# NVlabs/long-video-gan

Measured on NVIDIA H100. Metric: frames/sec (G+D train step: every convolution and torch_utils.ops call of the forward/backward passes, replayed), higher is better.
Workload: dtype f32

## Files before the change

### include/lvg_ops.h

```cpp
#ifndef LVG_OPS_H_
#define LVG_OPS_H_

#include <stdint.h>

#ifdef __cplusplus
extern "C" {
#endif

#define LVG_ABI_VERSION 2

#define LVG_OK            0
#define LVG_UNSUPPORTED (-1)
#define LVG_ERR_ARG       1
#define LVG_ERR_CUDA      2

#define LVG_F32 0
#define LVG_F16 1
#define LVG_F64 2

#define LVG_ACT_LINEAR   1
#define LVG_ACT_RELU     2
#define LVG_ACT_LRELU    3
#define LVG_ACT_TANH     4
#define LVG_ACT_SIGMOID  5
#define LVG_ACT_ELU      6
#define LVG_ACT_SELU     7
#define LVG_ACT_SOFTPLUS 8
#define LVG_ACT_SWISH    9

int         lvg_abi_version(void);
const char* lvg_last_error(void);
const char* lvg_build_info(void);
int64_t     lvg_launch_count(void);

int lvg_bias_act(const void* x, const void* b, const void* xref, const void* yref,
                 const void* dy, void* y, int dtype, int64_t n, int64_t size_b,
                 int64_t step_b, int grad, int act, float alpha, float gain,
                 float clamp, void* stream);

int lvg_bias_act_grad_db(const void* dy_in, const void* b, const void* xref,
                         const void* yref, void* dx, float* db_f32, int dtype,
                         int64_t n, int64_t size_b, int64_t step_b, int act,
                         float alpha, float gain, float clamp, void* stream);
int lvg_bias_act_fwd_codes(const void* x, const void* b, void* y, void* codes, int dtype, int64_t n,
                           int64_t size_b, int64_t step_b, int act, float alpha, float gain, float clamp,
                           void* stream);
int lvg_bias_act_bwd_codes(const void* dy, const void* codes, void* dx, float* db_f32, int dtype, int64_t n,
                           int64_t size_b, int64_t step_b, int act, float alpha, float gain, float clamp,
                           void* stream);
int64_t lvg_bias_act_codes_bytes(int dtype, int64_t n);

int lvg_upfirdn2d(const void* x, const float* f, void* y, int dtype,
                  const int64_t x_shape[4], const int64_t x_stride[4],
                  const int64_t y_shape[4], const int64_t y_stride[4],
                  int fw, int fh, int64_t f_stride_x, int64_t f_stride_y,
                  int upx, int upy, int downx, int downy, int padx0, int pady0,
                  int flip, float gain, void* stream);

int lvg_upfirdn2d_sep(const void* x, const float* fx, const float* fy, void* y,
                      int dtype, const int64_t x_shape[4], const int64_t x_stride[4],
                      const int64_t y_shape[4], const int64_t y_stride[4],
                      int fw, int fh, int upx, int upy, int downx, int downy,
                      int padx0, int pady0, int flip, float gain, void* stream);

int lvg_filtered_lrelu(const void* x, const float* fu, const float* fd, const void* b,
                       const uint8_t* si, void* y, uint8_t* so, int dtype,
                       const int64_t x_shape[4], const int64_t x_stride[4],
                       const int64_t y_shape[4], const int64_t y_stride[4],
                       int fu_w, int fu_h, int fd_w, int fd_h, int up, int down,
                       int px0, int py0, int s_h, int s_wbytes, int sx, int sy,
                       float gain, float slope, float clamp, int flip,
                       int write_signs, void* stream);

int lvg_filtered_lrelu_supported(int dtype, int fu_w, int fu_h, int fd_w, int fd_h,
                                 int up, int down);

int lvg_filtered_lrelu_act(void* x, const uint8_t* si, uint8_t* so, int dtype,
                           const int64_t x_shape[4], const int64_t x_stride[4],
                           int s_h, int s_wbytes, int sx, int sy, float gain,
                           float slope, float clamp, int write_signs, void* stream);

int lvg_fma(const void* a, const void* b, const void* c, void* out, int dtype,
            int rank, const int64_t shape[6], const int64_t a_stride[6],
            const int64_t b_stride[6], const int64_t c_stride[6], void* stream);

int64_t lvg_convnd_workspace(int dtype, int n, int groups, int cin, int cout, int t, int h, int wd,
                             int kt, int kh, int kw, int pad_t, int pad_h, int pad_w);
int lvg_convnd_fprop(const void* x, const void* w, void* y, int dtype, int n, int groups, int cin, int cout,
                     int t, int h, int wd, int kt, int kh, int kw, int pad_t, int pad_h, int pad_w, int stride,
                     const float* bias, int act, float alpha, float gain, float clamp,
                     void* workspace, int64_t workspace_bytes, void* stream);
int lvg_convnd_dgrad(const void* dy, const void* w, void* dx, int dtype, int n, int groups, int cin, int cout,
                     int t, int h, int wd, int kt, int kh, int kw, int pad_t, int pad_h, int pad_w, int stride,
                     void* workspace, int64_t workspace_bytes, void* stream);
int64_t lvg_convnd_wgrad_workspace(int dtype, int n, int groups, int cin, int cout, int t, int h, int wd,
                                   int kt, int kh, int kw, int pad_t, int pad_h, int pad_w);
int lvg_convnd_wgrad(const void* x, const void* dy, void* dw, int dtype, int n, int groups, int cin, int cout,
                     int t, int h, int wd, int kt, int kh, int kw, int pad_t, int pad_h, int pad_w, int stride,
                     void* workspace, int64_t workspace_bytes, void* stream);
int lvg_convnd_plan(int mode, int dtype, int n, int groups, int cin, int cout, int t, int h, int wd, int kt, int kh, int kw,
                    int pad_t, int pad_h, int pad_w, int stride, int* out, int out_len);
int lvg_convnd_epilogue_plan(int mode, int dtype, int n, int groups, int cin, int cout, int t, int h, int wd, int kt, int kh,
                             int kw, int pad_t, int pad_h, int pad_w, int stride, int* out, int out_len);
int lvg_convnd_route(int mode, int dtype, int n, int groups, int cin, int cout, int t, int h, int wd, int kt, int kh, int kw,
                     int pad_t, int pad_h, int pad_w, int stride, int epilogue);
int lvg_convnd_wgrad_plan(int dtype, int n, int groups, int cin, int cout, int t, int h, int wd, int kt, int kh, int kw,
                          int pad_t, int pad_h, int pad_w, int* out, int out_len);
int64_t lvg_convnd_backward_workspace(int dtype, int n, int groups, int cin, int cout, int t, int h, int wd,
                                      int kt, int kh, int kw, int pad_t, int pad_h, int pad_w);
int lvg_convnd_backward(const void* x, const void* dy, const void* w, void* dx, void* dw, int dtype, int n, int groups,
                        int cin, int cout, int t, int h, int wd, int kt, int kh, int kw, int pad_t, int pad_h, int pad_w,
                        int stride, void* workspace, int64_t workspace_bytes, void* stream);

int64_t lvg_modconv_workspace(int dtype, int n, int cin, int cout, int t, int h, int wd, int kt, int kh, int kw,
                              int pad_t, int pad_h, int pad_w);
int lvg_modconv_fprop(const void* x, const void* w, const float* a, const float* d, void* y, int dtype, int n, int cin,
                      int cout, int t, int h, int wd, int kt, int kh, int kw, int pad_t, int pad_h, int pad_w,
                      void* workspace, int64_t workspace_bytes, void* stream);
int lvg_modconv_backward(const void* x, const void* w, const float* a, const float* d, const void* y, const void* dy,
                         void* dx, void* dw, float* da, float* dyy, int dtype, int n, int cin, int cout, int t, int h,
                         int wd, int kt, int kh, int kw, int pad_t, int pad_h, int pad_w, void* workspace,
                         int64_t workspace_bytes, void* stream);

int64_t lvg_fir1d_depthwise_workspace(int groups);
int lvg_fir1d_depthwise(const float* x, const float* w, float* y, int n, int groups, int lin, int k,
                        void* workspace, int64_t workspace_bytes, void* stream);

int lvg_fir3d(const void* x, const float* f, void* y, int dtype, int n, int c, int t_in, int h_in, int w_in, int t_out,
              int h_out, int w_out, int filt_t, int filt_h, int filt_w, int step_t, int step_h, int step_w, int off_t,
              int off_h, int off_w, int fold, void* stream);
int lvg_fir3d_adjoint(const void* x, const float* f, void* y, int dtype, int n, int c, int t_in, int h_in, int w_in,
                      int t_out, int h_out, int w_out, int filt_t, int filt_h, int filt_w, int step_t, int step_h,
                      int step_w, int off_t, int off_h, int off_w, int fold, void* stream);

#define LVG_VIDEO_AUGMENT_LINEAR 1
int64_t lvg_video_augment_workspace(int n, int c, int t_in, int h, int w, int t_out);
int lvg_video_augment(const float* x, const float* params, float* y, void* workspace, int n, int c, int t_in, int h, int w,
                      int t_out, int flags, void* stream);
int lvg_video_augment_adjoint(const float* dy, const float* params, float* dx, void* workspace, int n, int c, int t_in,
                              int h, int w, int t_out, void* stream);

#define LVG_AUGMENT_PIPE_NPAR 23
#define LVG_AUGMENT_PIPE_GEOM 1
#define LVG_AUGMENT_PIPE_LINEAR 2
int64_t lvg_augment_pipe_workspace(int n, int c, int t, int h, int w, int flags);
int lvg_augment_pipe(const float* x, const float* params, const float* filter, int ntaps, const float* noise, float* y, int n,
                     int c, int t, int h, int w, int flags, void* stream);
int lvg_augment_pipe_adjoint(const float* dy, const float* params, const float* filter, int ntaps, float* dx, void* workspace,
                             int n, int c, int t, int h, int w, int flags, void* stream);

#define LVG_GBLOCK_TAIL_TUP 1
#define LVG_GBLOCK_TAIL_SUP 2
int64_t lvg_gblock_tail_workspace(int n, int c, int t, int h, int w, int t_out, int h_out, int w_out, int flags);
int lvg_gblock_tail(const void* s, const void* h, const float* b, void* z, uint8_t* codes, int dtype, int n, int c, int t,
                    int hh, int ww, int t_out, int h_out, int w_out, int flags, int act, float alpha, float gain, float clamp,
                    void* stream);
int lvg_gblock_tail_adjoint(const void* dz, const uint8_t* codes, void* dm, float* db, void* workspace, int64_t workspace_bytes,
                            int dtype, int n, int c, int t, int hh, int ww, int t_out, int h_out, int w_out, int flags, int act,
                            float alpha, float gain, void* stream);

#define LVG_DBLOCK_TAIL_TDOWN 1
#define LVG_DBLOCK_TAIL_SDOWN 2
#define LVG_DBLOCK_TAIL_MERGE 4
#define LVG_DBLOCK_TAIL_NONE 0
#define LVG_DBLOCK_TAIL_WRITE 1
#define LVG_DBLOCK_TAIL_READ 2
int64_t lvg_dblock_tail_workspace(int n, int c, int t, int h, int w, int flags);
int64_t lvg_dblock_tail_codes_bytes(int n, int c, int t, int h, int w, int flags);
int lvg_dblock_tail(const void* y, const void* s, const float* b, const float* f, void* z, uint8_t* codes, int mode, int dtype,
                    int n, int c, int t, int h, int w, int flags, int act, float alpha, float gain, float clamp, void* stream);
int lvg_dblock_tail_adjoint(const void* dz, const uint8_t* codes, const float* f, void* dy, void* ds, float* db, void* workspace,
                            int64_t workspace_bytes, int dtype, int n, int c, int t, int h, int w, int flags, int act,
                            float alpha, float gain, void* stream);

#define LVG_SRES_COND_NPLAN 10
int64_t lvg_sres_cond_workspace(int n, int t, int c, int c_lr, int window, int t_lr, int h_lr, int w_lr, int z_dtype,
                                const int* plan_h, const int* plan_w);
int lvg_sres_cond(const void* x, const float* lr, const float* f_h, const float* f_w, void* z, float* mean_sq, void* workspace,
                  int64_t workspace_bytes, int x_dtype, int z_dtype, int n, int t, int c, int c_lr, int window, int t_lr,
                  int h_lr, int w_lr, const int64_t* lr_strides, const int* plan_h, const int* plan_w, float gain_h,
                  float gain_w, void* stream);

int64_t lvg_sres_layer_workspace(int dtype, int n, int t, int c, int c_lr, int window, int t_lr, int h_lr, int w_lr,
                                 const int* plan_h, const int* plan_w, int cout, int kh, int kw, int pad_h, int pad_w);
int lvg_sres_layer_fprop(const void* x, const float* lr, const float* f_h, const float* f_w, const void* w, const float* a,
                         const float* d, void* y, float* mean_sq, int x_dtype, int dtype, int n, int t, int c, int c_lr,
                         int window, int t_lr, int h_lr, int w_lr, const int64_t* lr_strides, const int* plan_h,
                         const int* plan_w, float gain_h, float gain_w, int cout, int kh, int kw, int pad_h, int pad_w,
                         void* workspace, int64_t workspace_bytes, void* stream);
int lvg_sres_layer_backward(const void* x, const float* lr, const float* f_h, const float* f_w, const void* w, const float* a,
// ... 67 lines not shown
```

### long-video-gan_b200/csrc/conv_engine.cuh

```cuda
#pragma once

#include <cuda_bf16.h>

#include "common.cuh"

namespace lvg {

__device__ __forceinline__ unsigned short bf16_bits(float v) { return __bfloat16_as_ushort(__float2bfloat16_rn(v)); }
__device__ __forceinline__ float bf16_val(unsigned short b) { return __uint_as_float((uint32_t)b << 16); }

__device__ __forceinline__ float to_f32(float v) { return v; }
__device__ __forceinline__ float to_f32(__half v) { return __half2float(v); }
__device__ __forceinline__ void from_f32(float& o, float v) { o = v; }
__device__ __forceinline__ void from_f32(__half& o, float v) { o = __float2half_rn(v); }

inline int round_up(int a, int b) { return (a + b - 1) / b * b; }
inline int64_t round256(int64_t b) { return (b + 255) / 256 * 256; }

struct ConvShape {
    int dtype, n, groups, cin, cout, t, h, wd, kt, kh, kw, pad_t, pad_h, pad_w, stride;

    int split() const { return dtype == LVG_F32 ? 1 : 0; }
    int taps() const { return kt * kh * kw; }
    int64_t inst() const { return (int64_t)n * groups; }
    int64_t thw() const { return (int64_t)t * h * wd; }
    int to() const { return t + 2 * pad_t - kt + 1; }
    int ho() const { return h + 2 * pad_h - kh + 1; }
    int wo() const { return wd + 2 * pad_w - kw + 1; }
    int hos() const { return (ho() - 1) / stride + 1; }
    int wos() const { return (wo() - 1) / stride + 1; }
    bool empty() const { return to() < 1 || ho() < 1 || wo() < 1; }

    bool tileable() const;
    bool fprop_ok() const;
    bool dgrad_ok() const;
    bool wgrad_ok() const;
};

struct Geometry {
    int cpad, cblk, nblk, nimg, kc, mt;
    int m64, a_img;
    int64_t act_bytes, w_bytes;
};
Geometry geometry(int split, int64_t inst, int groups, int ck, int cm, int64_t thw, int taps);

struct ActGate {
    const void* y;
    int act;
    float alpha, gain, clamp;
};

struct IgemmJob {
    const void* x;
    const unsigned char* x8_pre;
    const float* in_scale;
    ActGate in_gate;
    int xin_h, xin_w, dil;
    int dtype, n, groups, ck, cm, t, h, wd, kt, kh, kw, pad_t, pad_h, pad_w;
    const void* w;
    int64_t gs, sm, sk;
    int flip;
    void* y;
    const float* bias;
    int act;
    float alpha, gain, clamp;
    const float* out_scale;
    int ostride;
};
IgemmJob fprop_job(const ConvShape& s, const void* x, const void* w, void* y);
IgemmJob dgrad_job(const ConvShape& s, const void* dy, const void* w, void* dx);

struct IgemmRooms {
    int64_t wp, x8;
    int64_t total() const { return wp + x8 + 256; }
};
IgemmRooms igemm_rooms(const IgemmJob& j);
int run_igemm(const IgemmJob& j, void* workspace, int64_t workspace_bytes, cudaStream_t s);

struct WgradPlan {
    int split, cpad_a, cpad_b, nt, ntiles, mt, nsplit;
    int ablk, khc, mrows;
    int nseg, seg_w[4], seg_x0[4], ps, rh, stages;
    int a_stage, b_stage, stage_bytes, tail_bytes;
    size_t smem;
    int64_t a_bytes, b_bytes, part_bytes, dw_elems;
};
WgradPlan wgrad_plan(const ConvShape& s, bool fold = true);

struct WgradInputs {
    const unsigned char* dy8_pre;
    const unsigned char* x8_pre;
    const float* x_scale;
    const float* dy_scale;
    ActGate dy_gate;
};

struct WgradRooms {
    int64_t dy8, x8, part;
    int64_t total() const { return dy8 + x8 + part + 512; }
};
WgradRooms wgrad_rooms(const WgradPlan& q, bool dy8_pre);
int run_wgrad(const ConvShape& s, const void* x, const void* dy, void* dw, const WgradInputs& in, void* workspace, int64_t workspace_bytes,
              cudaStream_t st);

struct BackwardRooms {
    int64_t dy8, rest;
    int64_t x8;
    int64_t total() const { return dy8 + rest; }
};
bool shares_dy8(const ConvShape& s);
BackwardRooms backward_rooms(const ConvShape& s, bool shared);
int64_t backward_workspace(const ConvShape& s);
struct Backward {
    const unsigned char* dy8;
    unsigned char* rest;
    int64_t rest_bytes;
    unsigned char* x8;
    ActGate gate;
};
int backward_dgrad(const ConvShape& s, const void* dy, const float* d, const void* w, void* dx, void* workspace, int64_t workspace_bytes,
                   cudaStream_t st, Backward& b, const ActGate* gate = nullptr);
int backward_wgrad(const ConvShape& s, const Backward& b, const void* x, const void* dy, const float* d, void* dw, const float* x_scale,
                   const unsigned char* x8_pre, cudaStream_t st);

bool modconv_in_envelope(const ConvShape& s);
int modconv_rowdot(void* u, const void* v, const float* scale, float* r, int dtype, int64_t rows, int64_t len, cudaStream_t s);

}
```

### long-video-gan_b200/csrc/conv_igemm.cu

```cuda

#include <algorithm>
#include <cuda.h>
#include <stdlib.h>
#include <type_traits>

#include "common.cuh"
#include "wgmma.cuh"
#include "conv_engine.cuh"

namespace lvg {
bool pw_supported(int dtype, int groups, int cin, int cout, int kt, int kh, int kw, int pad_t, int pad_h, int pad_w, int stride, int64_t P);
int pw_conv(const float* x, const float* w, float* y, int n, int cin, int cout, int64_t P, int64_t w_sco, int64_t w_sci, cudaStream_t s);
bool pw_tc_supported(int dtype, int groups, int cin, int cout, int kt, int kh, int kw, int pad_t, int pad_h, int pad_w, int stride, int64_t P);
int pw_tc_conv(const void* x, const void* w, void* y, int dtype, int n, int ck, int cm, int64_t P, int64_t w_sm, int64_t w_sk, void* workspace,
               int64_t workspace_bytes, cudaStream_t s, const void* res = nullptr, float rscale = 1.f);
int64_t pw_tc_workspace(int dtype, int ck, int cm);
}

namespace lvg {
namespace {

using namespace tc;

constexpr int kBM = 128;
// ... 827 lines not shown
    int nt;
    int nblk_a, nblk_b;
    int lo_a, lo_b;
    int nseg, seg_w[4], seg_x0[4], ps[4];
    int rh;
    int khc;
    int ablk;
    int nsplit;
    int a_bytes, b_bytes, stage_bytes, stages;
    int64_t split_stride;
    int mrows;
    int tail_bytes;
};

struct WgradMaps { CUtensorMap a[4]; CUtensorMap b; };

template <bool BF16, int TAPS, int NT>
__global__ void __launch_bounds__(kIgemmThreads, 1) conv_wgrad_v2_kernel(const __grid_constant__ WgradMaps maps, const WgradV2Params p)
{
    extern __shared__ __align__(128) unsigned char smem_raw[];
    __shared__ uint64_t full_bar[kMaxStages], empty_bar[kMaxStages];
    unsigned char* smem = reinterpret_cast<unsigned char*>((reinterpret_cast<uintptr_t>(smem_raw) + 127) & ~(uintptr_t)127);

    const int warp = threadIdx.x / 32, lane = threadIdx.x % 32;
    const int wg = __shfl_sync(0xffffffffu, (int)threadIdx.x / 128, 0);
    int bx = blockIdx.x;
    const int sp = bx % p.nsplit; bx /= p.nsplit;
    int ky0 = 0;
    if (p.khc == 1) { ky0 = bx % p.kh; bx /= p.kh; }
    const int kt = bx % p.kt;
    const int nti = bx / p.kt;
    const int mti = blockIdx.y, g = blockIdx.z;
    const int nop = p.split ? 2 : 1;
    const int consumers = p.mrows / 64;

    const int rblocks = (p.ho + p.rh - 1) / p.rh;
    const int per_plane = p.nseg * rblocks;
    const int total = p.n * p.to * per_plane;
    const int s0 = (int)((int64_t)total * sp / p.nsplit), s1 = (int)((int64_t)total * (sp + 1) / p.nsplit);

    if (threadIdx.x == 0) {
        for (int s = 0; s < p.stages; s++) { mbar_init(&full_bar[s], 1); mbar_init(&empty_bar[s], (uint32_t)consumers); }
        fence_barrier_init();
    }
    for (int i = threadIdx.x; i < (p.stages * p.stage_bytes + p.tail_bytes) / 16; i += kIgemmThreads) reinterpret_cast<uint4*>(smem)[i] = make_uint4(0u, 0u, 0u, 0u);
    fence_proxy_async();
    __syncthreads();

    if (wg == 0) {
        if (warp == 0 && elect_one()) {
            for (int s = s0; s < s1; s++) {
                const int it = s - s0, slot = it % p.stages;
                if (it >= p.stages) mbar_wait(&empty_bar[slot], (uint32_t)((it / p.stages - 1) & 1));
                int r = s;
                const int rb = r % rblocks; r /= rblocks;
                const int seg = r % p.nseg; r /= p.nseg;
                const int t = r % p.to;
                const int n = r / p.to;
                const int inst = n * p.groups + g;
                unsigned char* st = smem + (size_t)slot * p.stage_bytes;
                mbar_expect_tx(&full_bar[slot], (uint32_t)(nop * (p.a_bytes + p.b_bytes)));
                const int oy0 = rb * p.rh;
                for (int o = 0; o < nop; o++) {
                    tma_load_4d(st + (size_t)o * p.a_bytes, &maps.a[seg], 0, oy0, t, inst * p.nblk_a + o * p.lo_a + mti * 16, &full_bar[slot]);
                    tma_load_4d(st + (size_t)nop * p.a_bytes + (size_t)o * p.b_bytes, &maps.b, 2 * (p.seg_x0[seg] - p.pad_w), oy0 + ky0 - p.pad_h,
                                t + kt - p.pad_t, inst * p.nblk_b + o * p.lo_b + nti * (NT / 8), &full_bar[slot]);
                }
            }
        }
    } else if (wg >= 1 && wg - 1 < consumers) {
        const int cw = wg - 1;
        const int tid = threadIdx.x % 128, wq = tid / 32;
        float acc[TAPS][NT / 2];
#pragma unroll
        for (int tap = 0; tap < TAPS; tap++)
#pragma unroll
            for (int i = 0; i < NT / 2; i++) acc[tap][i] = 0.f;
        int prev = -1;
        for (int s = s0; s < s1; s++) {
            const int it = s - s0, slot = it % p.stages;
            const int seg = (s / rblocks) % p.nseg;
            const int rb = s % rblocks;
            const int rows = min(p.rh, p.ho - rb * p.rh);
            const int ksteps = (rows * p.ps[seg] + 15) / 16;
            const uint32_t blk_a = (uint32_t)(p.rh * p.ps[seg] * 16);
            const uint32_t blk_b = (uint32_t)((p.rh + p.khc - 1) * p.ps[seg] * 16);
            const uint32_t ky16 = (uint32_t)p.ps[seg];
            mbar_wait(&full_bar[slot], (uint32_t)((it / p.stages) & 1));
            wgmma_fence();
            const uint32_t a0 = smem_u32(smem + (size_t)slot * p.stage_bytes) + (uint32_t)cw * 8u * blk_a;
            const uint32_t b0 = smem_u32(smem + (size_t)slot * p.stage_bytes) + (uint32_t)(nop * p.a_bytes);
            const uint32_t a_hi = desc_hi(blk_a), b_hi = desc_hi(blk_b);
            for (int term = 0; term < (p.split ? 3 : 1); term++) {
                const uint32_t a_lo0 = desc_lo(a0 + (term == 1 ? (uint32_t)p.a_bytes : 0u), 128);
                const uint32_t b_lo0 = desc_lo(b0 + (term == 2 ? (uint32_t)p.b_bytes : 0u), 128);
                for (int k = 0; k < ksteps; k++) {
#pragma unroll
                    for (int tap = 0; tap < TAPS; tap++) {
                        const int kyi = tap / p.kw, kx = tap - kyi * p.kw;
                        wgmma_m64nNk16<BF16, NT, 1, 1>(acc[tap], a_lo0 + 16u * k, a_hi, b_lo0 + 16u * k + (uint32_t)kyi * ky16 + (uint32_t)kx, b_hi);
                    }
                }
            }
            wgmma_commit();
            wgmma_wait<1>();
            mbar_arrive_if(&empty_bar[prev >= 0 ? prev : 0], prev >= 0 && tid == 0);
            prev = slot;
        }
        wgmma_wait<0>();

        const int taps = p.kt * p.kh * p.kw;
        const int ci0 = nti * NT;
#pragma unroll
        for (int tap = 0; tap < TAPS; tap++) {
            const int kyi = tap / p.kw, kx = tap - kyi * p.kw;
            const int tapg = (kt * p.kh + ky0 + kyi) * p.kw + kx;
#pragma unroll
            for (int i = 0; i < NT / 2; i++) {
                const int co = mti * kBM + cw * 64 + wq * 16 + lane / 4 + 8 * ((i / 2) % 2);
                const int cil = (i / 4) * 8 + 2 * (lane % 4) + i % 2;
                if (co >= p.cout || ci0 + cil >= p.cin) continue;
                const int64_t off = (((int64_t)g * p.cout + co) * p.cin + ci0 + cil) * taps + tapg;
                const float v = acc[tap][i];
                if (p.nsplit > 1) reinterpret_cast<float*>(p.dw)[(int64_t)sp * p.split_stride + off] = v;
                else if (p.out_f32) reinterpret_cast<float*>(p.dw)[off] = v;
                else reinterpret_cast<__half*>(p.dw)[off] = __float2half_rn(v);
            }
        }
    }
}

template <class TOut>
__global__ void __launch_bounds__(256) conv_wgrad_reduce_kernel(const float* __restrict__ part, TOut* __restrict__ out, int64_t n, int nsplit, int64_t stride)
{
    for (int64_t i = (int64_t)blockIdx.x * blockDim.x + threadIdx.x; i < n; i += (int64_t)gridDim.x * blockDim.x) {
        float s = 0.f;
        for (int k = 0; k < nsplit; k++) s += part[(int64_t)k * stride + i];
        if constexpr (sizeof(TOut) == 2) out[i] = __float2half_rn(s);
        else out[i] = s;
    }
}

inline int wgrad_cpad_a(int cout) { return (cout < kBM && env_flag("LVG_WGRAD_COMPACT", 1)) ? round_up(cout, 16) : round_up(cout, kBM); }

}

WgradPlan wgrad_plan(const ConvShape& s, bool fold)
{
    const int cin = s.cin, cout = s.cout, kh = s.kh, kw = s.kw;
    const int to = s.to(), ho = s.ho(), wo = s.wo();
    WgradPlan q;
    q.split = s.split();
    q.cpad_a = wgrad_cpad_a(cout);
    q.ablk = q.cpad_a < kBM ? q.cpad_a / 8 : 16;
    q.mrows = (q.cpad_a <= 64 && env_flag("LVG_WGRAD_M64", 1)) ? 64 : kBM;
    q.cpad_b = round_up(cin, 16);
    q.khc = (fold && kh > 1 && kh * kw * 32 <= 256 && cin <= env_flag("LVG_WGRAD_FOLD_CIN", 32) && env_flag("LVG_WGRAD_FOLD", 1)) ? kh : 1;
    int nt_cap = (256 / (q.khc * kw)) / 32 * 32;
    if (q.split && nt_cap > 128) nt_cap = 128;
    q.nseg = (wo + 128 - kw) / (129 - kw);
    if (q.nseg < 1) q.nseg = 1;
    const int w0 = (wo + q.nseg - 1) / q.nseg;
    for (int j = 0; j < 4; j++) { q.seg_x0[j] = j * w0; q.seg_w[j] = j < q.nseg ? (wo - j * w0 < w0 ? wo - j * w0 : w0) : 0; }
    q.ps = round_up(w0 + kw - 1, 8);
    const int nop = q.split ? 2 : 1;
    auto stage_of = [&](int rows, int nt) { return nop * (q.ablk * rows + (nt / 8) * (rows + q.khc - 1)) * q.ps * 16; };
    {
        if (q.ps % 16 != 0 && 2 * stage_of(2, 64 < nt_cap ? 64 : nt_cap) > 200 * 1024) q.ps = round_up(q.ps, 16);
    }
    {
        const int min_rows = q.ps % 16 != 0 ? 2 : 1;
        while (nt_cap > 32 && 2 * stage_of(min_rows, nt_cap) > 200 * 1024) nt_cap -= 32;
    }
    q.ntiles = (q.cpad_b + nt_cap - 1) / nt_cap;
    q.nt = round_up((q.cpad_b + q.ntiles - 1) / q.ntiles, 32);
    q.cpad_b = q.nt * q.ntiles;
    q.mt = (q.cpad_a + kBM - 1) / kBM;
    const int64_t inst = s.inst();
    q.a_bytes = inst * nop * (q.cpad_a / 8) * (int64_t)to * ho * wo * 16;
    q.b_bytes = inst * nop * (q.cpad_b / 8) * s.thw() * 16;
    q.dw_elems = (int64_t)s.groups * cout * cin * s.taps();
    q.rh = 1;
    while (q.rh < ho && q.rh < 255 - q.khc && stage_of(q.rh + 1, q.nt) <= 80 * 1024) q.rh++;
    if (q.ps % 16 != 0) q.rh = q.rh >= 2 ? q.rh / 2 * 2 : 2;
    for (;;) {
// ... 207 lines not shown
    LVG_REQUIRE(x && dy && dw, "convnd_wgrad: x, dy, dw must not be NULL");
    const ConvShape sh = {dtype, n, groups, cin, cout, t, h, wd, kt, kh, kw, pad_t, pad_h, pad_w, stride};
    if (!sh.wgrad_ok()) {
        set_error("convnd_wgrad: outside the tensor-core kernel's envelope");
        return LVG_UNSUPPORTED;
    }
    return run_wgrad(sh, x, dy, dw, WgradInputs{}, workspace, workspace_bytes, (cudaStream_t)stream);
}

extern "C" int lvg_convnd_route(int mode, int dtype, int n, int groups, int cin, int cout, int t, int h, int wd, int kt, int kh, int kw, int pad_t,
                                int pad_h, int pad_w, int stride, int epilogue)
{
    const ConvShape sh = {dtype, n, groups, cin, cout, t, h, wd, kt, kh, kw, pad_t, pad_h, pad_w, stride};
    if (mode < 0 || mode > 2 || n < 1 || groups < 1) return LVG_UNSUPPORTED;
    if (mode == 2) return sh.wgrad_ok() ? 0 : LVG_UNSUPPORTED;
    if (mode == 1 || !epilogue) {
        if (pw_supported(dtype, groups, cin, cout, kt, kh, kw, pad_t, pad_h, pad_w, stride, sh.thw())) return 1;
        if (pw_tc_supported(dtype, groups, cin, cout, kt, kh, kw, pad_t, pad_h, pad_w, stride, sh.thw())) return 2;
    }
    return (mode == 0 ? sh.fprop_ok() : sh.dgrad_ok()) ? 0 : LVG_UNSUPPORTED;
}

extern "C" int lvg_convnd_plan(int mode, int dtype, int n, int groups, int cin, int cout, int t, int h, int wd, int kt, int kh, int kw, int pad_t,
                               int pad_h, int pad_w, int stride, int* out, int out_len)
{
    LVG_REQUIRE(out && out_len >= 48, "convnd_plan: out must hold 48 ints");
    LVG_REQUIRE(mode == 0 || mode == 1, "convnd_plan: mode 0 (forward) or 1 (input gradient)");
    const ConvShape sh = {dtype, n, groups, cin, cout, t, h, wd, kt, kh, kw, pad_t, pad_h, pad_w, stride};
    if (!(mode == 0 ? sh.fprop_ok() : sh.dgrad_ok())) {
        set_error("convnd_plan: outside the tensor-core kernel's envelope");
        return LVG_UNSUPPORTED;
    }
    for (int i = 0; i < out_len; i++) out[i] = 0;
    if (pw_supported(dtype, groups, cin, cout, kt, kh, kw, pad_t, pad_h, pad_w, stride, sh.thw())) { out[47] = 1; return LVG_OK; }
    if (mode == 1 && sh.empty()) { set_error("convnd_plan: empty output"); return LVG_UNSUPPORTED; }
    IgemmParams p;
    const int rc = plan_igemm(mode == 0 ? fprop_job(sh, nullptr, nullptr, nullptr) : dgrad_job(sh, nullptr, nullptr, nullptr), p);
    if (rc) return rc;
    const int v[48] = {p.wgroups, p.cout, p.mt, p.kc, p.nblk, p.nimg, p.lo_blk, p.to, p.ho, p.wo, p.kt, p.kh, p.kw, p.pad_t, p.pad_h, p.pad_w,
                       p.tt, p.th, p.wt, p.wtb, p.thb, p.frame_px, p.ncols, p.tiles_x, p.tiles_y, p.tiles_t,
                       (int)p.total_tiles, p.ks, p.stages, p.a_resident, p.a_stage, p.b_step, p.b_bytes, p.b_box, p.stage_bytes, p.ostride, p.hos, p.wos,
                       p.m64, p.ncw, 0, 0, 0, 0, 0, 0, 0, 0};
    for (int i = 0; i < 48; i++) out[i] = v[i];
    return LVG_OK;
}

extern "C" int lvg_convnd_epilogue_plan(int mode, int dtype, int n, int groups, int cin, int cout, int t, int h, int wd, int kt, int kh, int kw,
                                        int pad_t, int pad_h, int pad_w, int stride, int* out, int out_len)
{
    LVG_REQUIRE(out && out_len >= 4, "convnd_epilogue_plan: out must hold 4 ints");
    int plan[48];
    const int rc = lvg_convnd_plan(mode, dtype, n, groups, cin, cout, t, h, wd, kt, kh, kw, pad_t, pad_h, pad_w, stride, plan, 48);
    if (rc) return rc;
    for (int i = 0; i < out_len; i++) out[i] = 0;
    if (plan[47]) { out[0] = -1; return LVG_OK; }
    const ConvShape sh = {dtype, n, groups, cin, cout, t, h, wd, kt, kh, kw, pad_t, pad_h, pad_w, stride};
    IgemmParams p;
    const int prc = plan_igemm(mode == 0 ? fprop_job(sh, nullptr, nullptr, nullptr) : dgrad_job(sh, nullptr, nullptr, nullptr), p);
    if (prc) return prc;
    out[0] = p.pair_store;
    out[1] = p.stages;
    out[2] = igemm_smem_bytes(p);
    out[3] = kMapCols * (int)sizeof(int2);
    return LVG_OK;
}

extern "C" int lvg_convnd_wgrad_plan(int dtype, int n, int groups, int cin, int cout, int t, int h, int wd, int kt, int kh, int kw, int pad_t,
                                     int pad_h, int pad_w, int* out, int out_len)
{
    LVG_REQUIRE(out && out_len >= 32, "convnd_wgrad_plan: out must hold 32 ints");
    const ConvShape sh = {dtype, n, groups, cin, cout, t, h, wd, kt, kh, kw, pad_t, pad_h, pad_w, 1};
    if (!sh.wgrad_ok()) {
        set_error("convnd_wgrad_plan: outside the tensor-core kernel's envelope");
        return LVG_UNSUPPORTED;
    }
    const WgradPlan q = wgrad_plan(sh);
    const int v[32] = {q.split, q.cpad_a, q.cpad_b, q.nt, q.ntiles, q.mt, q.nsplit, q.ablk, q.khc, q.nseg, q.ps, q.rh, q.stages, q.a_stage, q.b_stage,
                       q.stage_bytes, q.tail_bytes, (int)q.smem, q.seg_w[0], q.seg_w[1], q.seg_w[2], q.seg_w[3], q.seg_x0[0], q.seg_x0[1], q.seg_x0[2],
                       q.seg_x0[3], 0, q.mrows, 0, 0, 0, 0};
    for (int i = 0; i < 32; i++) out[i] = v[i];
    return LVG_OK;
}

extern "C" int64_t lvg_convnd_backward_workspace(int dtype, int n, int groups, int cin, int cout, int t, int h, int wd, int kt, int kh, int kw,
                                                 int pad_t, int pad_h, int pad_w)
{
    const ConvShape sh = {dtype, n, groups, cin, cout, t, h, wd, kt, kh, kw, pad_t, pad_h, pad_w, 1};
    if (!sh.wgrad_ok()) return -1;
    return std::max(backward_workspace(sh), pw_tc_workspace(dtype, cout, cin));
}

extern "C" int lvg_convnd_backward(const void* x, const void* dy, const void* w, void* dx, void* dw, int dtype, int n, int groups, int cin, int cout,
                                   int t, int h, int wd, int kt, int kh, int kw, int pad_t, int pad_h, int pad_w, int stride, void* workspace,
                                   int64_t workspace_bytes, void* stream)
{
    LVG_REQUIRE(x && dy && w && dx && dw, "convnd_backward: x, dy, w, dx, dw must not be NULL");
    LVG_REQUIRE(workspace && aligned16(workspace), "convnd_backward: workspace must be 16-byte aligned and not NULL");
    const ConvShape sh = {dtype, n, groups, cin, cout, t, h, wd, kt, kh, kw, pad_t, pad_h, pad_w, stride};
    if (!sh.wgrad_ok() || !sh.dgrad_ok() || lvg_convnd_route(1, dtype, n, groups, cin, cout, t, h, wd, kt, kh, kw, pad_t, pad_h, pad_w, stride, 0) != 0) {
        const int rc = lvg_convnd_dgrad(dy, w, dx, dtype, n, groups, cin, cout, t, h, wd, kt, kh, kw, pad_t, pad_h, pad_w, stride, workspace,
                                        workspace_bytes, stream);
        if (rc) return rc;
        return lvg_convnd_wgrad(x, dy, dw, dtype, n, groups, cin, cout, t, h, wd, kt, kh, kw, pad_t, pad_h, pad_w, stride, workspace, workspace_bytes,
                                stream);
    }
    cudaStream_t s = (cudaStream_t)stream;
    Backward b;
    const int rc = backward_dgrad(sh, dy, nullptr, w, dx, workspace, workspace_bytes, s, b);
    if (rc) return rc;
    return backward_wgrad(sh, b, x, dy, nullptr, dw, nullptr, nullptr, s);
}
```

### long-video-gan_b200/torch_utils/custom_ops.py

```python
import ctypes
import math
import os

import torch

from .ops._util import is_absent, is_dense

verbosity = 'brief'

_LIB_NAME = 'liblvg_ops.so'
_lib = None
_plugins = {}

_c_void_p = ctypes.c_void_p
_c_int = ctypes.c_int
_c_i64 = ctypes.c_int64
_c_float = ctypes.c_float
_I64x4 = ctypes.c_int64 * 4
_I64x6 = ctypes.c_int64 * 6

_DTYPE_CODE = {torch.float32: 0, torch.float16: 1, torch.float64: 2}

_SIGNATURES = {
    'lvg_abi_version': (_c_int, []),
    'lvg_last_error': (ctypes.c_char_p, []),
    'lvg_build_info': (ctypes.c_char_p, []),
    'lvg_launch_count': (_c_i64, []),
    'lvg_grad_postprocess': (_c_int, [_c_void_p, _c_i64, _c_float, _c_float, _c_void_p]),
    'lvg_adam_step': (_c_int, [_c_void_p] * 5 + [_c_i64] + [_c_float] * 4 + [_c_i64, _c_float, _c_float, _c_int, _c_float, _c_void_p]),
    'lvg_lerp': (_c_int, [_c_void_p, _c_void_p, _c_i64, _c_float, _c_void_p]),
    'lvg_bias_act': (_c_int, [_c_void_p] * 6 + [_c_int, _c_i64, _c_i64, _c_i64, _c_int, _c_int, _c_float, _c_float, _c_float, _c_void_p]),
    'lvg_bias_act_grad_db': (_c_int, [_c_void_p] * 6 + [_c_int, _c_i64, _c_i64, _c_i64, _c_int, _c_float, _c_float, _c_float, _c_void_p]),
    'lvg_bias_act_fwd_codes': (_c_int, [_c_void_p] * 4 + [_c_int, _c_i64, _c_i64, _c_i64, _c_int, _c_float, _c_float, _c_float, _c_void_p]),
    'lvg_bias_act_codes_bytes': (_c_i64, [_c_int, _c_i64]),
    'lvg_bias_act_bwd_codes': (_c_int, [_c_void_p] * 4 + [_c_int, _c_i64, _c_i64, _c_i64, _c_int, _c_float, _c_float, _c_float, _c_void_p]),
    'lvg_upfirdn2d': (_c_int, [_c_void_p, _c_void_p, _c_void_p, _c_int, _I64x4, _I64x4, _I64x4, _I64x4, _c_int, _c_int, _c_i64, _c_i64]
                      + [_c_int] * 7 + [_c_float, _c_void_p]),
    'lvg_upfirdn2d_sep': (_c_int, [_c_void_p] * 4 + [_c_int, _I64x4, _I64x4, _I64x4, _I64x4] + [_c_int] * 9 + [_c_float, _c_void_p]),
    'lvg_filtered_lrelu': (_c_int, [_c_void_p] * 7 + [_c_int, _I64x4, _I64x4, _I64x4, _I64x4] + [_c_int] * 12
                           + [_c_float, _c_float, _c_float, _c_int, _c_int, _c_void_p]),
    'lvg_filtered_lrelu_supported': (_c_int, [_c_int] * 7),
    'lvg_filtered_lrelu_act': (_c_int, [_c_void_p] * 3 + [_c_int, _I64x4, _I64x4] + [_c_int] * 4 + [_c_float] * 3 + [_c_int, _c_void_p]),
    'lvg_fma': (_c_int, [_c_void_p] * 4 + [_c_int, _c_int, _I64x6, _I64x6, _I64x6, _I64x6, _c_void_p]),
    'lvg_fir1d_depthwise_workspace': (_c_i64, [_c_int]),
    'lvg_fir1d_depthwise': (_c_int, [_c_void_p] * 3 + [_c_int] * 4 + [_c_void_p, _c_i64, _c_void_p]),
    'lvg_convnd_workspace': (_c_i64, [_c_int] * 14),
    'lvg_convnd_fprop': (_c_int, [_c_void_p] * 3 + [_c_int] * 15 + [_c_void_p, _c_int, _c_float, _c_float, _c_float, _c_void_p, _c_i64, _c_void_p]),
    'lvg_convnd_dgrad': (_c_int, [_c_void_p] * 3 + [_c_int] * 15 + [_c_void_p, _c_i64, _c_void_p]),
    'lvg_convnd_wgrad_workspace': (_c_i64, [_c_int] * 14),
    'lvg_convnd_wgrad': (_c_int, [_c_void_p] * 3 + [_c_int] * 15 + [_c_void_p, _c_i64, _c_void_p]),
    'lvg_convnd_plan': (_c_int, [_c_int] * 16 + [ctypes.POINTER(_c_int), _c_int]),
    'lvg_convnd_epilogue_plan': (_c_int, [_c_int] * 16 + [ctypes.POINTER(_c_int), _c_int]),
    'lvg_convnd_wgrad_plan': (_c_int, [_c_int] * 14 + [ctypes.POINTER(_c_int), _c_int]),
    'lvg_convnd_route': (_c_int, [_c_int] * 17),
    'lvg_convnd_backward_workspace': (_c_i64, [_c_int] * 14),
    'lvg_convnd_backward': (_c_int, [_c_void_p] * 5 + [_c_int] * 15 + [_c_void_p, _c_i64, _c_void_p]),
    'lvg_modconv_workspace': (_c_i64, [_c_int] * 13),
    'lvg_modconv_fprop': (_c_int, [_c_void_p] * 5 + [_c_int] * 13 + [_c_void_p, _c_i64, _c_void_p]),
    'lvg_modconv_backward': (_c_int, [_c_void_p] * 10 + [_c_int] * 13 + [_c_void_p, _c_i64, _c_void_p]),
    'lvg_fir3d': (_c_int, [_c_void_p] * 3 + [_c_int] * 19 + [_c_void_p]),
    'lvg_fir3d_adjoint': (_c_int, [_c_void_p] * 3 + [_c_int] * 19 + [_c_void_p]),
    'lvg_video_augment_workspace': (_c_i64, [_c_int] * 6),
    'lvg_video_augment': (_c_int, [_c_void_p] * 4 + [_c_int] * 7 + [_c_void_p]),
    'lvg_video_augment_adjoint': (_c_int, [_c_void_p] * 4 + [_c_int] * 6 + [_c_void_p]),
    'lvg_augment_pipe_workspace': (_c_i64, [_c_int] * 6),
    'lvg_augment_pipe': (_c_int, [_c_void_p] * 3 + [_c_int] + [_c_void_p] * 2 + [_c_int] * 6 + [_c_void_p]),
    'lvg_augment_pipe_adjoint': (_c_int, [_c_void_p] * 3 + [_c_int] + [_c_void_p] * 2 + [_c_int] * 6 + [_c_void_p]),
    'lvg_gblock_tail_workspace': (_c_i64, [_c_int] * 9),
    'lvg_gblock_tail': (_c_int, [_c_void_p] * 5 + [_c_int] * 11 + [_c_float] * 3 + [_c_void_p]),
    'lvg_gblock_tail_adjoint': (_c_int, [_c_void_p] * 5 + [_c_i64] + [_c_int] * 11 + [_c_float] * 2 + [_c_void_p]),
    'lvg_dblock_tail_workspace': (_c_i64, [_c_int] * 6),
    'lvg_dblock_tail_codes_bytes': (_c_i64, [_c_int] * 6),
    'lvg_dblock_tail': (_c_int, [_c_void_p] * 6 + [_c_int] * 9 + [_c_float] * 3 + [_c_void_p]),
    'lvg_dblock_tail_adjoint': (_c_int, [_c_void_p] * 7 + [_c_i64] + [_c_int] * 8 + [_c_float] * 2 + [_c_void_p]),
    'lvg_sres_cond_workspace': (_c_i64, [_c_int] * 9 + [_c_void_p] * 2),
    'lvg_sres_cond': (_c_int, [_c_void_p] * 7 + [_c_i64] + [_c_int] * 10 + [_c_void_p] * 3 + [_c_float] * 2 + [_c_void_p]),
    'lvg_sres_layer_workspace': (_c_i64, [_c_int] * 9 + [_c_void_p] * 2 + [_c_int] * 5),
    'lvg_sres_layer_fprop': (_c_int, [_c_void_p] * 9 + [_c_int] * 10 + [_c_void_p] * 3 + [_c_float] * 2 + [_c_int] * 5
                             + [_c_void_p, _c_i64, _c_void_p]),
    'lvg_sres_layer_backward': (_c_int, [_c_void_p] * 13 + [_c_int] * 10 + [_c_void_p] * 3 + [_c_float] * 2 + [_c_int] * 5
                                + [_c_void_p, _c_i64, _c_void_p]),
    'lvg_sres_torgb_workspace': (_c_i64, [_c_int] * 9 + [_c_void_p] * 2 + [_c_int]),
    'lvg_sres_torgb_fprop': (_c_int, [_c_void_p] * 9 + [_c_int] * 10 + [_c_void_p] * 3 + [_c_float] * 2 + [_c_int, _c_float, _c_void_p]),
    'lvg_sres_torgb_backward': (_c_int, [_c_void_p] * 12 + [_c_int] * 10 + [_c_void_p] * 3 + [_c_float] * 2 + [_c_int]
                                + [_c_void_p, _c_i64, _c_void_p]),
    'lvg_lres_torgb_workspace': (_c_i64, [_c_int] * 11),
    'lvg_lres_torgb_fprop': (_c_int, [_c_void_p] * 7 + [_c_int] * 8 + [_c_float, _c_void_p, _c_i64, _c_void_p]),
    'lvg_lres_torgb_finish': (_c_int, [_c_void_p] * 4 + [_c_int] * 5 + [_c_float, _c_void_p]),
    'lvg_lres_torgb_backward': (_c_int, [_c_void_p] * 9 + [_c_int] * 8 + [_c_float, _c_void_p, _c_i64, _c_void_p]),
    'lvg_gblock_conv0_workspace': (_c_i64, [_c_int] * 13),
    'lvg_gblock_conv0_fprop': (_c_int, [_c_void_p] * 7 + [_c_int] * 14 + [_c_float] * 3 + [_c_void_p, _c_i64, _c_void_p]),
    'lvg_gblock_conv0_backward': (_c_int, [_c_void_p] * 12 + [_c_int] * 14 + [_c_float] * 3 + [_c_void_p, _c_i64, _c_void_p]),
    'lvg_sres_dblock_conv1_workspace': (_c_i64, [_c_int] * 6),
    'lvg_sres_dblock_conv1': (_c_int, [_c_void_p] * 3 + [_c_int] + [_c_void_p] * 3 + [_c_int] * 7 + [_c_float] * 3 + [_c_void_p, _c_i64, _c_void_p]),
    'lvg_sres_dblock_conv1_backward_workspace': (_c_i64, [_c_int] * 6),
    'lvg_sres_dblock_conv1_backward': (_c_int, [_c_void_p] * 3 + [_c_int] + [_c_void_p] * 4 + [_c_int] * 6 + [_c_void_p, _c_i64, _c_void_p]),
    'lvg_sres_dblock_fir_adjoint_act_workspace': (_c_i64, [_c_int] * 5),
    'lvg_sres_dblock_fir_adjoint_act': (_c_int, [_c_void_p] * 4 + [_c_int] + [_c_void_p] * 3 + [_c_i64] + [_c_int] * 6 + [_c_float] * 3 + [_c_void_p]),
    'lvg_sres_dblock_skip_workspace': (_c_i64, [_c_int] * 4 + [_c_i64]),
    'lvg_sres_dblock_skip': (_c_int, [_c_void_p] * 4 + [_c_int] * 4 + [_c_i64, _c_float, _c_void_p, _c_i64, _c_void_p]),
}

LVG_UNSUPPORTED = -1


def library_path():
    return os.path.join(os.path.dirname(os.path.dirname(os.path.abspath(__file__))), _LIB_NAME)


def load_library():
    global _lib
    if _lib is None:
        path = os.environ.get('LVG_OPS_LIBRARY', library_path())
        if not os.path.isfile(path):
            raise RuntimeError(
                f'{_LIB_NAME} not found at {path}: build it with `python -c "import __graft_entry__ as g; g.build()"` '
                f'or `make -C long-video-gan_b200/csrc`. There is no fallback for CUDA tensors.')
        lib = ctypes.CDLL(path)
        for name, (restype, argtypes) in _SIGNATURES.items():
            fn = getattr(lib, name)
            fn.restype = restype
            fn.argtypes = argtypes
        if lib.lvg_abi_version() != 2:
            raise RuntimeError(f'{path}: unexpected ABI version {lib.lvg_abi_version()}')
        _lib = lib
    return _lib


def exported_symbols():
    return sorted(_SIGNATURES)


def launch_count():
    return int(load_library().lvg_launch_count())


# ... 1123 lines not shown
```

Measured before the change: 2429.

## Skip padded columns in wgrad K-walk using split-stride wgmma descriptors

The wgrad tensor-core loop used to step through each row's padded pitch in 16-element chunks, so MMAs also ran over the padding columns. It now walks only the 8-column groups that cover the real segment width, jumping past the padding at row ends. Each k16 step is built from two 8-element halves, with their offset encoded as the descriptor's leading-byte stride (swizzle field changed from 128 to 0). A host-side ksteps query is exported for testing. The risks are descriptor-layout correctness and some extra index arithmetic in the inner loop.

After: 2527 (median of 6 runs). +4.0%, better.

```diff
diff --git a/include/lvg_ops.h b/include/lvg_ops.h
--- a/include/lvg_ops.h
+++ b/include/lvg_ops.h
@@ -106,6 +106,8 @@
                      int pad_t, int pad_h, int pad_w, int stride, int epilogue);
 int lvg_convnd_wgrad_plan(int dtype, int n, int groups, int cin, int cout, int t, int h, int wd, int kt, int kh, int kw,
                           int pad_t, int pad_h, int pad_w, int* out, int out_len);
+int lvg_convnd_wgrad_ksteps(int dtype, int n, int groups, int cin, int cout, int t, int h, int wd, int kt, int kh, int kw,
+                            int pad_t, int pad_h, int pad_w, int rows, int seg, int* out, int out_len);
 int64_t lvg_convnd_backward_workspace(int dtype, int n, int groups, int cin, int cout, int t, int h, int wd,
                                       int kt, int kh, int kw, int pad_t, int pad_h, int pad_w);
 int lvg_convnd_backward(const void* x, const void* dy, const void* w, void* dx, void* dw, int dtype, int n, int groups,
diff --git a/long-video-gan_b200/csrc/conv_engine.cuh b/long-video-gan_b200/csrc/conv_engine.cuh
--- a/long-video-gan_b200/csrc/conv_engine.cuh
+++ b/long-video-gan_b200/csrc/conv_engine.cuh
@@ -87,6 +87,29 @@
 };
 WgradPlan wgrad_plan(const ConvShape& s, bool fold = true);
 
+struct WgradKWalk {
+    int gw, skip, left;
+    int c;
+    uint32_t off;
+};
+__host__ __device__ __forceinline__ WgradKWalk wgrad_kwalk(int rows, int width, int ps)
+{
+    const int gw = (width + 7) / 8;
+    return {gw, ps - 8 * gw, rows * gw, 0, 0u};
+}
+__host__ __device__ __forceinline__ int wgrad_ksteps(const WgradKWalk& w) { return (w.left + 1) / 2; }
+__host__ __device__ __forceinline__ uint32_t wgrad_kstep(WgradKWalk& w)
+{
+    const uint32_t first = w.off;
+    w.off += 8;
+    if (++w.c == w.gw) { w.c = 0; w.off += (uint32_t)w.skip; }
+    const uint32_t second = w.left == 1 ? first + 8u : w.off;
+    w.off += 8;
+    if (++w.c == w.gw) { w.c = 0; w.off += (uint32_t)w.skip; }
+    w.left -= 2;
+    return first | (second - first) << 16;
+}
+
 struct WgradInputs {
     const unsigned char* dy8_pre;
     const unsigned char* x8_pre;
diff --git a/long-video-gan_b200/csrc/conv_igemm.cu b/long-video-gan_b200/csrc/conv_igemm.cu
--- a/long-video-gan_b200/csrc/conv_igemm.cu
+++ b/long-video-gan_b200/csrc/conv_igemm.cu
@@ -933,7 +933,8 @@
             const int seg = (s / rblocks) % p.nseg;
             const int rb = s % rblocks;
             const int rows = min(p.rh, p.ho - rb * p.rh);
-            const int ksteps = (rows * p.ps[seg] + 15) / 16;
+            const int width = p.seg_w[seg];
+            const int ksteps = wgrad_ksteps(wgrad_kwalk(rows, width, p.ps[seg]));
             const uint32_t blk_a = (uint32_t)(p.rh * p.ps[seg] * 16);
             const uint32_t blk_b = (uint32_t)((p.rh + p.khc - 1) * p.ps[seg] * 16);
             const uint32_t ky16 = (uint32_t)p.ps[seg];
@@ -943,15 +944,20 @@
             const uint32_t b0 = smem_u32(smem + (size_t)slot * p.stage_bytes) + (uint32_t)(nop * p.a_bytes);
             const uint32_t a_hi = desc_hi(blk_a), b_hi = desc_hi(blk_b);
             for (int term = 0; term < (p.split ? 3 : 1); term++) {
-                const uint32_t a_lo0 = desc_lo(a0 + (term == 1 ? (uint32_t)p.a_bytes : 0u), 128);
-                const uint32_t b_lo0 = desc_lo(b0 + (term == 2 ? (uint32_t)p.b_bytes : 0u), 128);
-                for (int k = 0; k < ksteps; k++) {
+                const uint32_t a_lo0 = desc_lo(a0 + (term == 1 ? (uint32_t)p.a_bytes : 0u), 0);
+                const uint32_t b_lo0 = desc_lo(b0 + (term == 2 ? (uint32_t)p.b_bytes : 0u), 0);
+                WgradKWalk walk = wgrad_kwalk(rows, width, p.ps[seg]);
+                auto mma_step = [&](uint32_t step) {
 #pragma unroll
                     for (int tap = 0; tap < TAPS; tap++) {
                         const int kyi = tap / p.kw, kx = tap - kyi * p.kw;
-                        wgmma_m64nNk16<BF16, NT, 1, 1>(acc[tap], a_lo0 + 16u * k, a_hi, b_lo0 + 16u * k + (uint32_t)kyi * ky16 + (uint32_t)kx, b_hi);
+                        wgmma_m64nNk16<BF16, NT, 1, 1>(acc[tap], a_lo0 + step, a_hi, b_lo0 + step + (uint32_t)kyi * ky16 + (uint32_t)kx, b_hi);
                     }
-                }
+                };
+                if (walk.skip == 0)
+                    for (int k = 0; k < ksteps; k++) mma_step(16u * k | 8u << 16);
+                else
+                    for (int k = 0; k < ksteps; k++) mma_step(wgrad_kstep(walk));
             }
             wgmma_commit();
             wgmma_wait<1>();
@@ -1325,6 +1331,28 @@
     return LVG_OK;
 }
 
+extern "C" int lvg_convnd_wgrad_ksteps(int dtype, int n, int groups, int cin, int cout, int t, int h, int wd, int kt, int kh, int kw, int pad_t,
+                                       int pad_h, int pad_w, int rows, int seg, int* out, int out_len)
+{
+    const ConvShape sh = {dtype, n, groups, cin, cout, t, h, wd, kt, kh, kw, pad_t, pad_h, pad_w, 1};
+    if (!sh.wgrad_ok()) {
+        set_error("convnd_wgrad_ksteps: outside the tensor-core kernel's envelope");
+        return LVG_UNSUPPORTED;
+    }
+    const WgradPlan q = wgrad_plan(sh);
+    LVG_REQUIRE(rows >= 1 && rows <= q.rh && seg >= 0 && seg < q.nseg, "convnd_wgrad_ksteps: rows in [1, %d], seg in [0, %d)", q.rh, q.nseg);
+    WgradKWalk w = wgrad_kwalk(rows, q.seg_w[seg], q.ps);
+    const int steps = wgrad_ksteps(w);
+    LVG_REQUIRE(out && out_len >= 1 + 2 * steps, "convnd_wgrad_ksteps: out must hold %d ints", 1 + 2 * steps);
+    out[0] = steps;
+    for (int k = 0; k < steps; k++) {
+        const uint32_t step = wgrad_kstep(w);
+        out[1 + 2 * k] = (int)(step & 0xffffu);
+        out[2 + 2 * k] = (int)(step >> 16);
+    }
+    return LVG_OK;
+}
+
 extern "C" int64_t lvg_convnd_backward_workspace(int dtype, int n, int groups, int cin, int cout, int t, int h, int wd, int kt, int kh, int kw,
                                                  int pad_t, int pad_h, int pad_w)
 {
diff --git a/long-video-gan_b200/torch_utils/custom_ops.py b/long-video-gan_b200/torch_utils/custom_ops.py
--- a/long-video-gan_b200/torch_utils/custom_ops.py
+++ b/long-video-gan_b200/torch_utils/custom_ops.py
@@ -52,6 +52,7 @@
     'lvg_convnd_plan': (_c_int, [_c_int] * 16 + [ctypes.POINTER(_c_int), _c_int]),
     'lvg_convnd_epilogue_plan': (_c_int, [_c_int] * 16 + [ctypes.POINTER(_c_int), _c_int]),
     'lvg_convnd_wgrad_plan': (_c_int, [_c_int] * 14 + [ctypes.POINTER(_c_int), _c_int]),
+    'lvg_convnd_wgrad_ksteps': (_c_int, [_c_int] * 16 + [ctypes.POINTER(_c_int), _c_int]),
     'lvg_convnd_route': (_c_int, [_c_int] * 17),
     'lvg_convnd_backward_workspace': (_c_i64, [_c_int] * 14),
     'lvg_convnd_backward': (_c_int, [_c_void_p] * 5 + [_c_int] * 15 + [_c_void_p, _c_i64, _c_void_p]),
```
